# chriscoey/Hypatia.jl

Hardware: AMD Instinct MI355X
Metric: IPM iterations/sec (+ ms per KKT solve): dense n=5000, PosSemidefTri side 200 (Float64, QRCholDense + CombinedStepper) (higher is better)
Workload: dtype f64

## Files before the change

### hypatia.jl_amd/_lib.py

```python
import ctypes
import os

import numpy as np

HERE = os.path.dirname(os.path.abspath(__file__))
LIB_PATH = os.environ.get("HYP_LIB_PATH") or os.path.join(HERE, "libhypatia_hip.so")

c_int, c_dbl, c_vp = ctypes.c_int, ctypes.c_double, ctypes.c_void_p
P = ctypes.POINTER

_lib = None
_ctx = None


class HypatiaHipError(RuntimeError):
    pass


SIGNATURES = {
    "hyp_ctx_create": [c_int, P(c_vp)],
    "hyp_ctx_destroy": [c_vp],
    "hyp_ctx_synchronize": [c_vp],
    "hyp_device_count": [P(c_int)],
    "hyp_get_timers": [c_vp, c_vp],
# ... 58 lines not shown
    "hyp_sys_step_directions": [c_vp, c_vp, c_vp, c_dbl, c_dbl, c_int, c_dbl, c_dbl, c_vp, c_vp, P(c_int), P(c_int), P(c_int), P(c_int), c_vp],
    "hyp_sys_set_comm": [c_vp, c_vp, c_vp, c_vp, ctypes.c_long],
    "hyp_comm_unique_id": [c_vp],
    "hyp_comm_init_rank": [c_vp, c_int, c_int, c_vp, P(c_vp)],
    "hyp_comm_destroy": [c_vp],
    "hyp_comm_allreduce": [c_vp, c_vp, ctypes.c_long, c_int],
    "hyp_sys_set_comm_rccl": [c_vp, c_vp],
    "hyp_sys_comm_stats": [c_vp, c_vp],
    "hyp_qrcp_factor": [c_vp, c_int, c_int, c_vp, c_int, c_vp, P(c_vp)],
    "hyp_qrcp_get": [c_vp, c_vp, c_vp, c_vp, c_vp],
    "hyp_qrcp_apply_q": [c_vp, c_int, c_vp],
    "hyp_qrcp_destroy": [c_vp],
    "hyp_sys_set_kshard": [c_vp, c_int, c_int],
    "hyp_sys_set_direction_rows": [c_vp, c_int],
    "hyp_sys_last_update_lhs_seconds": [c_vp, P(c_dbl)],
    "hyp_sys_bench_gemv": [c_vp, c_int, c_vp],
    "hyp_sys_search_alpha": [c_vp, c_vp, c_vp, c_vp, c_vp, c_vp, c_int, c_int, c_vp, c_int, c_int, c_dbl, c_dbl, c_int, c_dbl, c_vp,
                             P(c_int), P(c_dbl), P(c_int), P(c_int), P(c_dbl)],
    "hyp_sys_search_screen_stats": [c_vp, P(c_int), c_vp, c_vp],
    "hyp_sys_search_alpha_resident": [c_vp, c_int, c_int, c_vp, c_int, c_int, c_dbl, c_dbl, c_int, c_dbl, c_vp,
                                      P(c_int), P(c_dbl), P(c_int), P(c_int), P(c_dbl)],
    "hyp_sys_check_cone_points": [c_vp, c_vp, c_dbl, c_dbl, c_int, c_dbl, P(c_int), P(c_dbl), P(c_int), P(c_dbl)],
    "hyp_sys_residual_products": [c_vp, c_vp, c_vp, c_vp, c_vp, c_vp, c_vp],
    "hyp_sys_residual_products2": [c_vp, c_vp, c_vp, c_vp, c_dbl, c_vp, c_vp, c_vp, c_vp],
    "hyp_sys_set_comm_layout": [c_vp, c_int, c_int],
    "hyp_sys_comm_hist": [c_vp, c_vp],
    "hyp_sys_comm_times": [c_vp, c_vp],
    "hyp_sys_allreduce_host": [c_vp, c_vp, c_int, c_int],
    "hyp_sys_load_model": [c_vp, c_vp, c_vp, c_vp, c_vp],
    "hyp_sys_update_lhs": [c_vp, P(c_int), P(c_int), P(c_int), c_vp],
    "hyp_sys_get_directions": [c_vp, c_vp, c_vp, c_dbl, c_dbl, c_int, c_dbl, c_dbl, P(c_dbl), P(c_int)],
    "hyp_sys_assemble_lhs": [c_vp, P(c_int)],
    "hyp_sys_factor_lhs": [c_vp, P(c_int), P(c_int)],
    "hyp_sys_lhs_export_dev": [c_vp, c_vp],
    "hyp_sys_lhs_import_dev": [c_vp, c_vp],
    "hyp_sys_set_lhs": [c_vp, c_vp],
    "hyp_sys_potrs": [c_vp, c_vp],
    "hyp_sys_block_hess_prod": [c_vp, c_vp, c_vp],
    "hyp_sys_mul_G": [c_vp, c_int, c_dbl, c_vp, c_dbl, c_vp],
    "hyp_sys_get_lhs": [c_vp, c_vp],
    "hyp_dense_gemm": [c_vp, c_int, c_int, c_int, c_int, c_int, c_dbl, c_vp, c_int, c_vp, c_int, c_dbl, c_vp, c_int],
    "hyp_dense_syrk": [c_vp, c_int, c_int, c_vp, c_int, c_vp, c_int],
    "hyp_dense_potrf": [c_vp, c_int, c_vp, c_int, P(c_int)],
    "hyp_dense_posdef_solve": [c_vp, c_int, c_vp, c_int, c_vp, c_int, c_int, P(c_int), P(c_int), P(c_int)],
    "hyp_dense_posv": [c_vp, c_int, c_vp, c_int, c_vp, P(c_int)],
    "hyp_dense_posv_multi": [c_vp, c_int, c_vp, c_int, c_vp, c_int, c_int, P(c_int)],
    "hyp_dense_sysv_rook": [c_vp, c_int, c_vp, c_int, c_vp, c_int, c_int, P(c_int), c_vp, c_vp, c_vp, c_vp],
    "hyp_dense_lstsq_normal": [c_vp, c_int, c_int, c_vp, c_int, c_vp, c_vp, P(c_dbl), P(c_int)],
    "hyp_dense_gemv": [c_vp, c_int, c_int, c_int, c_dbl, c_vp, c_int, c_vp, c_dbl, c_vp],
    "hyp_dense_gemv_both": [c_vp, c_int, c_int, c_int, c_vp, c_int, c_vp, c_dbl, c_vp, c_vp, c_dbl, c_vp, P(c_int)],
    "hyp_bench_syrk": [c_vp, c_int, c_int, c_int, P(c_dbl)],
    "hyp_bench_potrf": [c_vp, c_int, c_int, P(c_dbl)],
    "hyp_bench_trsv": [c_vp, c_int, c_int, P(c_dbl), P(c_dbl)],
}


def load_library():
    global _lib
    if _lib is not None:
        return _lib
    if not os.path.exists(LIB_PATH):
        raise HypatiaHipError("libhypatia_hip.so is missing at %s: run __graft_entry__.build() "
                              "(hipcc --offload-arch=gfx950); there is no CPU fallback" % LIB_PATH)
    lib = ctypes.CDLL(LIB_PATH)
    for name, argtypes in SIGNATURES.items():
        fn = getattr(lib, name)
        fn.argtypes = argtypes
        fn.restype = c_int
    lib.hyp_last_error.argtypes = [c_vp]
    lib.hyp_last_error.restype = ctypes.c_char_p
    if os.environ.get("HYP_PROFILE"):
        lib = _ProfiledLib(lib)
    _lib = lib
    return lib


class _ProfiledLib:

    def __init__(self, lib):
        import time
        self._lib = lib
        self.stats = {}
        self._time = time.perf_counter

    def __getattr__(self, name):
        fn = getattr(self._lib, name)
        if not name.startswith("hyp_") or name == "hyp_last_error":
            return fn
        stats, clock = self.stats, self._time

        def wrapped(*a):
            t0 = clock()
            r = fn(*a)
            st = stats.setdefault(name, [0, 0.0])
            st[0] += 1
            st[1] += clock() - t0
            return r
        wrapped.__name__ = name
        setattr(self, name, wrapped)
        return wrapped

    def report(self):
        rows = sorted(self.stats.items(), key=lambda kv: -kv[1][1])
        return "\n".join("%-36s calls %6d  total %9.3f ms  avg %8.1f us" % (k, v[0], v[1] * 1e3, v[1] / v[0] * 1e6) for k, v in rows)

    def reset(self):
# ... 52 lines not shown
```

### hypatia.jl_amd/csrc/capi.hip

```cpp
#include <unistd.h>
#include "../../include/hypatia_hip.h"
#include "syssolver.hpp"
#include <chrono>
#include <cstring>

using namespace hyp;

struct hyp_ctx { Ctx c; hyp_ctx(int d) : c(d) {} };
struct hyp_cone { hyp_ctx* ctx; Cone* cone; };
struct hyp_sys { hyp_ctx* ctx; SysSolver* s; };
struct hyp_symindef { hyp_ctx* ctx; SymIndefSys* s; };
struct hyp_comm { hyp_ctx* ctx; void* nccl; int nranks, rank; };
namespace hyp {
struct QrcpFact;
QrcpFact* qrcp_create(Ctx& c, int m, int n, const double* hA, int lda, const double* hb);
void qrcp_get(QrcpFact* f, int* jpvt, double* R, double* rdiag, double* qtb);
void qrcp_apply_q(QrcpFact* f, bool trans, double* hx);
void qrcp_destroy(QrcpFact* f);
}
struct hyp_qrcp { hyp_ctx* ctx; hyp::QrcpFact* f; };

namespace hyp {
void rccl_allreduce_inplace(void* comm, double* d_buf, long count, int op, hipStream_t st);
void rccl_unique_id(char* out128);
// ... 1096 lines not shown
      const double v = (double)(s >> 11) * (1.0 / 9007199254740992.0) - 0.5;
      h[j * n + i] = h[i * n + j] = (i == j) ? (double)n : v;
    }
  for (auto& v : hx) { s ^= s << 13; s ^= s >> 7; s ^= s << 17; v = (double)(s >> 11) * (1.0 / 9007199254740992.0) - 0.5; }
  c.h2d(dA.p, h.data(), h.size() * 8);
  c.h2d(dx0.p, hx.data(), hx.size() * 8);
  potrf_upper_batched(c, n, dA.d(), n, 0, 1, dinv.d(), dinfo.i());
  c.d2h(c.h_info, dinfo.p, sizeof(int));
  c.sync();
  HYP_REQUIRE(c.h_info[0] == 0, "bench_trsv: factorization failed");
  hipEvent_t e0, e1;
  HYP_CHECK(hipEventCreate(&e0)); HYP_CHECK(hipEventCreate(&e1));
  TriSolvePlan tri;
  float tb = 0, t1 = 0, t2 = 0, t3 = 0;
  for (int r = 0; r <= reps; ++r) {
    float ms = 0;
    tri.invalidate();
    HYP_CHECK(hipEventRecord(e0, c.stream));
    tri.build(c, n, dA.d(), n, dinv.d());
    HYP_CHECK(hipEventRecord(e1, c.stream));
    HYP_CHECK(hipEventSynchronize(e1));
    HYP_CHECK(hipEventElapsedTime(&ms, e0, e1));
    if (r > 0) tb += ms;
    c.d2d(dx.p, dx0.p, (size_t)3 * n * 8);
    HYP_CHECK(hipEventRecord(e0, c.stream));
    tri.solve_both(c, dA.d(), n, dx.d(), n, 1);
    HYP_CHECK(hipEventRecord(e1, c.stream));
    HYP_CHECK(hipEventSynchronize(e1));
    HYP_CHECK(hipEventElapsedTime(&ms, e0, e1));
    if (r > 0) t1 += ms;
    if (x_out && r == reps) c.d2h(x_out, dx.p, (size_t)n * 8);
    c.d2d(dx.p, dx0.p, (size_t)3 * n * 8);
    HYP_CHECK(hipEventRecord(e0, c.stream));
    tri.solve_both(c, dA.d(), n, dx.d(), n, 2);
    HYP_CHECK(hipEventRecord(e1, c.stream));
    HYP_CHECK(hipEventSynchronize(e1));
    HYP_CHECK(hipEventElapsedTime(&ms, e0, e1));
    if (r > 0) t2 += ms;
    if (x_out && r == reps) c.d2h(x_out + n, dx.p, (size_t)2 * n * 8);
    c.d2d(dx.p, dx0.p, (size_t)3 * n * 8);
    HYP_CHECK(hipEventRecord(e0, c.stream));
    tri.solve_both(c, dA.d(), n, dx.d(), n, 3);
    HYP_CHECK(hipEventRecord(e1, c.stream));
    HYP_CHECK(hipEventSynchronize(e1));
    HYP_CHECK(hipEventElapsedTime(&ms, e0, e1));
    if (r > 0) t3 += ms;
    if (x_out && r == reps) c.d2h(x_out + 3 * n, dx.p, (size_t)3 * n * 8);
  }
  c.sync();
  ms_out4[0] = tb / reps; ms_out4[1] = t1 / reps; ms_out4[2] = t2 / reps; ms_out4[3] = t3 / reps;
  (void)hipEventDestroy(e0); (void)hipEventDestroy(e1);
  API_END(ctx)
}
int hyp_bench_syrk(hyp_ctx* ctx, int N, int K, int reps, double* ms_out) {
  API_BEGIN
  Ctx& c = ctx->c;
  DBuf dA((size_t)K * N * 8), dC((size_t)N * N * 8);
  std::vector<double> h((size_t)K * N);
  uint64_t s = 88172645463325252ULL;
  for (auto& v : h) { s ^= s << 13; s ^= s >> 7; s ^= s << 17; v = (double)(s >> 11) * (1.0 / 9007199254740992.0) * 2.0 - 1.0; }
  c.h2d(dA.p, h.data(), h.size() * 8);
  c.sync();
  GemmArgs g{};
  g.M = N; g.N = N; g.K = K; g.A = dA.d(); g.lda = K; g.B = dA.d(); g.ldb = K; g.C = dC.d(); g.ldc = N;
  g.alpha = 1; g.beta = 0; g.tri = GEMM_UPPER; g.krange = KR_ALL; g.batch = 1; g.tag = 1;
  gemm(c, true, g);
  c.sync();
  hipEvent_t e0, e1;
  HYP_CHECK(hipEventCreate(&e0)); HYP_CHECK(hipEventCreate(&e1));
  float ms = 0;
  const char* gap = getenv("HYP_BENCH_SYRK_GAP_US");
  if (gap && atoi(gap) > 0) {
    for (int r = 0; r < reps; ++r) {
      c.sync();
      usleep(atoi(gap));
      HYP_CHECK(hipEventRecord(e0, c.stream));
      gemm(c, true, g);
      HYP_CHECK(hipEventRecord(e1, c.stream));
      const char* burst = getenv("HYP_BENCH_SYRK_BURST");
      const int nb = burst ? std::min(atoi(burst), 8) : 0;
      hipEvent_t eb[9];
      for (int b = 0; b < nb; ++b) {
        gemm(c, true, g);
        HYP_CHECK(hipEventCreate(&eb[b]));
        HYP_CHECK(hipEventRecord(eb[b], c.stream));
      }
      HYP_CHECK(hipEventSynchronize(nb ? eb[nb - 1] : e1));
      float t = 0;
      HYP_CHECK(hipEventElapsedTime(&t, e0, e1));
      ms += t;
      if (nb) {
        fprintf(stderr, "burst after %s us idle: %.3f", gap, t);
        for (int b = 0; b < nb; ++b) {
          float tb = 0;
          HYP_CHECK(hipEventElapsedTime(&tb, b ? eb[b - 1] : e1, eb[b]));
          fprintf(stderr, " %.3f", tb);
        }
        fprintf(stderr, " ms\n");
        for (int b = 0; b < nb; ++b) (void)hipEventDestroy(eb[b]);
      }
    }
  } else {
    HYP_CHECK(hipEventRecord(e0, c.stream));
    for (int r = 0; r < reps; ++r) gemm(c, true, g);
    HYP_CHECK(hipEventRecord(e1, c.stream));
    HYP_CHECK(hipEventSynchronize(e1));
// ... 9 lines not shown
```

### hypatia.jl_amd/csrc/dense.hip

```cpp
#include <malloc.h>
#include "tds_small.hpp"
#include "hyp_internal.hpp"

#include <fcntl.h>
#include <sys/file.h>
#include <sys/stat.h>
#include <unistd.h>

namespace hyp {

void gemm(Ctx& c, bool transa, GemmArgs a) { HYP_CHECK(gemm_f64_launch(c.stream, transa, a, &c.gemm_scratch)); }

void potrf_diag_launch(hipStream_t st, bool factor, bool invert, int batch, int nblocks, double* A, long lda, long strideA, int n, int k0,
                       double* dinv, long strideD, int* info, int own_cu_lds = 0);
int potrf_diag_own_cu_lds();
void potrf_panel_solve_launch(hipStream_t st, int batch, double* A, long lda, long strideA, int k0, int mcols);
void potrf_diag_mfma_launch(hipStream_t st, int batch, double* A, long lda, long strideA, int n, int k0, int* info, int own_cu_lds,
                            double* tinv = nullptr, long tinv_stride = 0, bool prev_update = false);
bool potrf_tinv_on();
bool potrf_diag_prev_ok();
int potrf_diag_mfma_own_cu_lds();
void potrf_panel_mfma_launch(hipStream_t st, int batch, double* A, long lda, long strideA, int k0, int mcols, int coff = 0,
                             const double* tinv = nullptr, long tinv_stride = 0);

// ... 792 lines not shown
      for (int g = 0; g < 4; ++g) {
        Rs[(rowA + 4 * g) * 16 + li] = rA[g];
        Rs[(rowB + 4 * g) * 16 + li] = rB[g];
      }
      __syncthreads();
      tdr_product<LOWER>(dop, nb, wv, Rs, xA, xB);
    }
    __syncthreads();
#pragma unroll
    for (int g = 0; g < 4; ++g) {
      Xs[(rowA + 4 * g) * 16 + li] = xA[g];
      Xs[(rowB + 4 * g) * 16 + li] = xB[g];
    }
    __syncthreads();
    for (int e = tid; e < NB * 16; e += 256) {
      const int k = e & (NB - 1), c = e >> 7;
      if (k < nb && c0 + c < nrhs) X[(long)(c0 + c) * ldx + k] = Xs[k * 16 + c];
    }
    __syncthreads();
  }
}

void trsm_upper_left_fwd_batched(Ctx& c, int n, int nrhs, const double* U, long ldu, long strideU, const double* dinv, long strideD,
                                 double* X, long ldx, long strideX, int batch) {
  if (n <= 0 || nrhs <= 0 || batch <= 0) return;
  const int nblk = (n + NB - 1) / NB;
  const int refine = std::max(1, trsm_refine_steps());
  for (int kb = 0; kb < nblk; ++kb) {
    const int k0 = kb * NB, nb = std::min(NB, n - k0), m = n - k0 - nb;
    hipLaunchKernelGGL(trsm_diag_refined_fwd_batched_kernel, dim3((nrhs + 16 * TDR_CH - 1) / (16 * TDR_CH), batch), dim3(256), 0, c.stream, U + (long)k0 * ldu + k0, ldu,
                       strideU, dinv + (long)kb * DINV_BLK, strideD, nb, X + k0, ldx, strideX, nrhs, refine);
    HYP_CHECK(hipGetLastError());
    if (m > 0) {
      GemmArgs u{};
      u.M = m; u.N = nrhs; u.K = nb; u.A = U + (long)(k0 + nb) * ldu + k0; u.lda = ldu; u.strideA = strideU;
      u.B = X + k0; u.ldb = ldx; u.strideB = strideX; u.C = X + k0 + nb; u.ldc = ldx; u.strideC = strideX;
      u.alpha = -1; u.beta = 1; u.batch = batch;
      gemm(c, true, u);
    }
  }
}

__global__ void place_dinv_kernel(const double* __restrict__ dinv, long strideD, double* __restrict__ Uinv, long ldi, long strideI,
                                  int n) {
  const int b = blockIdx.z;
  const int l = blockIdx.y;
  const int i = blockIdx.x * blockDim.x + threadIdx.x;
  if (i >= n || l >= n) return;
  double v = 0.0;
  if (i / NB == l / NB) v = dinv[(long)b * strideD + (long)(l / NB) * DINV_BLK + (long)(l % NB) * NB + (i % NB)];
  Uinv[(long)b * strideI + (long)l * ldi + i] = v;
}

void trtri_upper_batched(Ctx& c, int n, const double* U, long ldu, long strideU, const double* dinv, long strideD, double* Uinv,
                         long ldi, long strideI, int batch, DBuf* ws_override) {
  if (n <= 0 || batch <= 0) return;
  hipLaunchKernelGGL(place_dinv_kernel, dim3((n + 127) / 128, n, batch), dim3(128), 0, c.stream, dinv, strideD, Uinv, ldi, strideI, n);
  HYP_CHECK(hipGetLastError());
  const int nblk = (n + NB - 1) / NB;
  if (nblk == 1) return;
  DBuf& ws = ws_override ? *ws_override : c.work_tri;
  ws.ensure((size_t)batch * n * NB * sizeof(double));
  for (int jb = 1; jb < nblk; ++jb) {
    const int j0 = jb * NB, nb = std::min(NB, n - j0);
    GemmArgs t{};
    t.M = j0; t.N = nb; t.K = nb; t.A = U + (long)j0 * ldu; t.lda = ldu; t.strideA = strideU;
    t.B = dinv + (long)jb * DINV_BLK; t.ldb = NB; t.strideB = strideD;
    t.C = ws.d(); t.ldc = n; t.strideC = (long)n * NB; t.alpha = 1; t.beta = 0; t.krange = KR_LE_N; t.batch = batch;
    gemm(c, false, t);
    GemmArgs u{};
    u.M = j0; u.N = nb; u.K = j0; u.A = Uinv; u.lda = ldi; u.strideA = strideI;
    u.B = ws.d(); u.ldb = n; u.strideB = (long)n * NB;
    u.C = Uinv + (long)j0 * ldi; u.ldc = ldi; u.strideC = strideI; u.alpha = -1; u.beta = 0; u.krange = KR_GE_M; u.batch = batch;
    gemm(c, false, u);
  }
}

__global__ __launch_bounds__(256) void coldot_kernel(int m, int ncols, int mode, const double* __restrict__ M, long ld,
                                                     const double* __restrict__ v, const double* base, double alpha, double* out) {
  const int j = blockIdx.x * 4 + (threadIdx.x >> 6);
  if (j >= ncols) return;
  const int lane = threadIdx.x & 63;
  int i0 = 0, i1 = m;
  if (mode == 1) i1 = min(j + 1, m);
  else if (mode == 2) i0 = min(j, m);
  const double* a = M + (long)j * ld;
  double s0 = 0.0, s1 = 0.0, s2 = 0.0, s3 = 0.0;
  int i = i0 + lane;
  for (; i + 192 < i1; i += 256) {
    const double a0 = a[i], a1 = a[i + 64], a2 = a[i + 128], a3 = a[i + 192];
    s0 += a0 * v[i];
    s1 += a1 * v[i + 64];
    s2 += a2 * v[i + 128];
    s3 += a3 * v[i + 192];
  }
  for (; i < i1; i += 64) s0 += a[i] * v[i];
  double s = (s0 + s1) + (s2 + s3);
#pragma unroll
  for (int off = 32; off > 0; off >>= 1) s += __shfl_down(s, off);
  if (lane == 0) out[j] = (base ? base[j] : 0.0) + alpha * s;
}

__global__ __launch_bounds__(256) void coldot_batched_kernel(int m, int ncols, int mode, const double* __restrict__ M, long ld,
                                                             const double* __restrict__ v, const double* base, double alpha, double* out) {
  const int j = blockIdx.x * 4 + (threadIdx.x >> 6);
  if (j >= ncols) return;
  const int lane = threadIdx.x & 63;
  int i0 = 0, i1 = m;
// ... 62 lines not shown
    const double v1 = phase == 0 ? ((i & 1) ? -1.0 : 1.0) : t[n + r0 + i];
    s0 = fma(a, v0, s0);
    s1 = fma(a, v1, s1);
  }
#pragma unroll
  for (int off = 32; off > 0; off >>= 1) {
    s0 += __shfl_down(s0, off);
    s1 += __shfl_down(s1, off);
  }
  if (lane != 0) return;
  if (phase == 0) {
    t[J] = s0;
    t[n + J] = s1;
  } else {
    const double e0 = fabs(1.0 - s0), e1 = fabs(((j & 1) ? -1.0 : 1.0) - s1);
    double m = e0 > e1 ? e0 : e1;
    if (!(e0 == e0) || !(e1 == e1)) m = __longlong_as_double(0x7ff8000000000000LL);
    atomicMax(out, (unsigned long long)__double_as_longlong(m));
  }
}

void TriSolvePlan::measure_quality(Ctx& c, const double* U, long ldu) {
  probe_ws.ensure((size_t)(2 * n + 2) * sizeof(double));
  double* t = probe_ws.d();
  unsigned long long* out = reinterpret_cast<unsigned long long*>(t + 2 * n);
  c.zero(out, sizeof(unsigned long long));
  const dim3 grid((n + 3) / 4), blk(256);
  hipLaunchKernelGGL(plan_probe_kernel, grid, blk, 0, c.stream, 0, n, sb, Binv.d(), U, ldu, t, out);
  hipLaunchKernelGGL(plan_probe_kernel, grid, blk, 0, c.stream, 1, n, sb, Binv.d(), U, ldu, t, out);
  HYP_CHECK(hipGetLastError());
  c.d2h(c.h_pinned + 200, out, sizeof(double));
  c.sync();
  rho = c.h_pinned[200];
}

void TriSolvePlan::build(Ctx& c, int n_, const double* U, long ldu, const double* dinv) {
  n = 0;
  sb = c.trsv_plan_sb(n_);
  static const int refine_env = [] { const char* e = getenv("HYP_TRSV_REFINE"); return e ? atoi(e) : -1; }();
  refine_req = refine_env >= 0 ? refine_env : 2;
  refine = refine_req;
  rho = -1.0;
  if (sb <= 0 || n_ <= 0) return;
  const int nsb = (n_ + sb - 1) / sb;
  const size_t blk = (size_t)sb * sb;
  Binv.ensure(nsb * blk * sizeof(double));
  BinvT.ensure(nsb * blk * sizeof(double));
  UT.ensure((size_t)n_ * n_ * sizeof(double));
  work.ensure((size_t)2 * sb * sizeof(double));
  const int nfull = n_ / sb, last = n_ - nfull * sb;
  const long strideU = (long)sb * (ldu + 1), strideD = (long)(sb / NB) * DINV_BLK;
  const bool split = (nfull > 0 && last > 0);
  hipEvent_t e0 = c.aux_event(0), e1 = c.aux_event(1);
  if (split) {
    work2.ensure((size_t)last * NB * sizeof(double));
    HYP_CHECK(hipEventRecord(e0, c.stream));
    HYP_CHECK(hipStreamWaitEvent(c.stream2, e0, 0));
    {
      StreamSwap on_helper(c);
      dev_transpose(c, n_, n_, U, ldu, UT.d(), n_, 1, 0, 0);
      trtri_upper_batched(c, last, U + (long)nfull * strideU, ldu, 0, dinv + (long)nfull * strideD, 0, Binv.d() + nfull * blk, sb, 0, 1, &work2);
      dev_transpose(c, last, last, Binv.d() + nfull * blk, sb, BinvT.d() + nfull * blk, sb, 1, 0, 0);
      HYP_CHECK(hipEventRecord(e1, c.stream));
    }
  }
  if (nfull > 0) trtri_upper_batched(c, sb, U, ldu, strideU, dinv, strideD, Binv.d(), sb, (long)blk, nfull);
  if (!split && last > 0) {
    trtri_upper_batched(c, last, U + (long)nfull * strideU, ldu, 0, dinv + (long)nfull * strideD, 0, Binv.d() + nfull * blk, sb, 0, 1);
    dev_transpose(c, last, last, Binv.d() + nfull * blk, sb, BinvT.d() + nfull * blk, sb, 1, 0, 0);
  }
  if (nfull > 0) dev_transpose(c, sb, sb, Binv.d(), sb, BinvT.d(), sb, nfull, (long)blk, (long)blk);
  if (!split) dev_transpose(c, n_, n_, U, ldu, UT.d(), n_, 1, 0, 0);
  if (split) HYP_CHECK(hipStreamWaitEvent(c.stream, e1, 0));
  n = n_;
  static const int adapt_sel = [] { const char* e = getenv("HYP_TRSV_ADAPT"); return e ? atoi(e) : 3; }();
  const bool adapt = adapt_sel == 1 || (adapt_sel == 2 && owner_class == 0) || (adapt_sel == 3 && owner_class == 1);
  static const double adapt_tol = [] { const char* e = getenv("HYP_TRSV_ADAPT_TOL"); return e ? atof(e) : 1e-10; }();
  ++c.plan_builds;
  if (adapt && refine_req >= 2) {
    measure_quality(c, U, ldu);
    static const bool dbg = [] { const char* e = getenv("HYP_TRSV_ADAPT_DBG"); return e && e[0] == '1'; }();
    if (dbg) fprintf(stderr, "[solve plan] n = %d, super-blocks of %d: rho = %.3e\n", n, sb, rho);
    if (rho == rho && rho <= adapt_tol) { refine = 1; ++c.plan_builds_one_step; }
  }
  ol_prepare(c, ldu);
}

void TriSolvePlan::solve(Ctx& c, const double* U, long ldu, bool trans, double* x) {
  if (ol_usable(c, ldu, 1)) { ol_sweep(c, U, trans ? 0 : 1, x, 0, nullptr, 1); return; }
  const int nsb = (n + sb - 1) / sb;
  const size_t blk = (size_t)sb * sb;
  double* t = work.d();
  double* e = work.d() + sb;
  for (int s = 0; s < nsb; ++s) {
    const int b = trans ? s : nsb - 1 - s;
    const int r0 = b * sb, m = std::min(sb, n - r0);
    double* xb = x + r0;
    const double* Dm = trans ? U + (long)r0 * ldu + r0 : UT.d() + (long)r0 * n + r0;
    const long ldd = trans ? ldu : n;
    const double* Bm = (trans ? Binv.d() : BinvT.d()) + b * blk;
    const int mode = trans ? 1 : 2;
    if (refine == 0) {
      coldot(c, m, m, mode, Bm, sb, xb, nullptr, 1.0, t);
      HYP_CHECK(hipMemcpyAsync(xb, t, (size_t)m * sizeof(double), hipMemcpyDeviceToDevice, c.stream));
    } else {
      coldot(c, m, m, mode, Bm, sb, xb, nullptr, 1.0, t);
      for (int it = 0; it < refine; ++it) {
        coldot(c, m, m, mode, Dm, ldd, t, xb, -1.0, e);
        coldot(c, m, m, mode, Bm, sb, e, t, 1.0, it + 1 == refine ? xb : t);
      }
    }
    if (trans) {
      const int rest = n - (r0 + m);
      coldot(c, m, rest, 0, U + (long)(r0 + m) * ldu + r0, ldu, xb, x + r0 + m, -1.0, x + r0 + m);
    } else {
      coldot(c, m, r0, 0, UT.d() + r0, n, xb, x, -1.0, x);
    }
  }
  HYP_CHECK(hipGetLastError());
}

template <int NC>
__global__ __launch_bounds__(256) void coldotn_kernel(int m, int ncols, int mode, const double* __restrict__ M, long ld,
                                                      const double* __restrict__ v, long ldv, const double* base, long ldb, double alpha,
                                                      double* out, long ldo) {
  const int j = blockIdx.x * 4 + (threadIdx.x >> 6);
// ... 422 lines not shown
```

### hypatia.jl_amd/csrc/hyp_internal.hpp

```cpp
#pragma once
#include <hip/hip_runtime.h>
#include <stdint.h>
#include <string>
#include <vector>
#include <utility>
#include <stdexcept>
#include "gemm_f64.hpp"

namespace hyp {

struct HipError : std::runtime_error {
  int code;
  HipError(int c, const std::string& m) : std::runtime_error(m), code(c) {}
};

#define HYP_CHECK(expr)                                                                         \
  do {                                                                                          \
    hipError_t e_ = (expr);                                                                     \
    if (e_ != hipSuccess)                                                                       \
      throw hyp::HipError(-(int)e_ - 1000, std::string(#expr) + ": " + hipGetErrorString(e_) +  \
                                                " at " __FILE__ ":" + std::to_string(__LINE__)); \
  } while (0)

#define HYP_REQUIRE(cond, msg)                                                     \
// ... 117 lines not shown
  }
};

struct StreamSwap {
  Ctx& c;
  explicit StreamSwap(Ctx& ctx) : c(ctx) { std::swap(c.stream, c.stream2); std::swap(c.gemm_scratch, c.gemm_scratch2); std::swap(c.potrf_tinv, c.potrf_tinv2); }
  ~StreamSwap() { std::swap(c.stream, c.stream2); std::swap(c.gemm_scratch, c.gemm_scratch2); std::swap(c.potrf_tinv, c.potrf_tinv2); }
  StreamSwap(const StreamSwap&) = delete;
  StreamSwap& operator=(const StreamSwap&) = delete;
};

struct Ctx::Lane {
  hipStream_t s = nullptr;
  GemmScratch gs;
  DBuf tinv;
  hipEvent_t done = nullptr;
};

struct LaneSwitch {
  Ctx& c;
  int i;
  explicit LaneSwitch(Ctx& ctx, int lane) : c(ctx), i(lane) { flip(); }
  ~LaneSwitch() { flip(); }
  LaneSwitch(const LaneSwitch&) = delete;
  LaneSwitch& operator=(const LaneSwitch&) = delete;
 private:
  void flip() {
    if (i == 1) { std::swap(c.stream, c.stream2); std::swap(c.gemm_scratch, c.gemm_scratch2); std::swap(c.potrf_tinv, c.potrf_tinv2); }
    else if (i >= 2) { Ctx::Lane& L = c.lane(i); std::swap(c.stream, L.s); std::swap(c.gemm_scratch, L.gs); std::swap(c.potrf_tinv, L.tinv); }
  }
};
void fork_lanes(Ctx& c, int nlanes);
void join_lanes(Ctx& c, int nlanes);


void potrf_upper_batched(Ctx& c, int n, double* A, long lda, long strideA, int batch, double* dinv, int* d_info, int kb_stop = -1);
bool potrf_split_ok(int n, int n1);
void schur_split_begin(Ctx& c, int n, int K, const double* A, long lda, double* C, double* F, int n1, int* d_info, hipStream_t lane,
                       hipEvent_t left_ready, hipEvent_t left_done);
void schur_split_finish(Ctx& c, int n, const double* C, double* F, int n1, double* dinv, int* d_info, hipEvent_t left_done);
void potrf_invert_diag_blocks(Ctx& c, int n, double* A , long lda, long strideA, int batch, double* dinv,
                              long strideD = 0 );
constexpr long DINV_BLK = 2L * NB * NB;
inline size_t dinv_elems(int n) { return (size_t)((n + NB - 1) / NB) * DINV_BLK; }

void trsv_upper(Ctx& c, int n, const double* U, long ldu, const double* dinv, bool trans, double* x);
int trsm_refine_steps();
void trsm_upper_left(Ctx& c, int n, int nrhs, const double* U, long ldu, const double* dinv, bool trans, double* X,
                     long ldx, double* work );
void trsm_upper_left_fwd_batched(Ctx& c, int n, int nrhs, const double* U, long ldu, long strideU, const double* dinv, long strideD,
                                 double* X, long ldx, long strideX, int batch);
struct TriSolvePlan {
  int n = 0, sb = 0, refine = 2;
  DBuf Binv, BinvT, UT, work, work2, work_n;
  bool ready(int n_) const { return n == n_ && n_ > 0; }
  void invalidate() { n = 0; }
  void build(Ctx& c, int n_, const double* U, long ldu, const double* dinv);
  DBuf ol_rounds[4], ol_arena;
  bool ol_ok = false;
  bool ol_have[4] = {false, false, false, false};
  int ol_n = 0, ol_sb = 0, ol_set = 0;
  long ol_ldu = 0, ol_asz = 0;
  int ol_first[4][3] = {}, ol_n0[4][3] = {}, ol_n1[4][3] = {};
  void ol_prepare(Ctx& c, long ldu);
  int refine_req = 2;
  int owner_class = 0;
  double rho = -1.0;
  DBuf probe_ws;
  void measure_quality(Ctx& c, const double* U, long ldu);
  bool ol_fit[4] = {false, false, false, false};
  static bool ol_fits(Ctx& c, int nr);
  bool ol_usable(const Ctx& c, long ldu, int nr) const { return ol_ok && nr >= 1 && nr <= 3 && ol_fit[nr] && c.persistent_ok && refine >= 0 && refine <= 3 && ol_have[refine] && ldu == ol_ldu && c.stream == c.stream_primary; }
  void ol_sweep(Ctx& c, const double* U, int which, double* x, long ldx, double* x3, int nr);
  void solve_both(Ctx& c, const double* U, long ldu, double* x, long ldx, int nr, double* x3 = nullptr);
  void solve(Ctx& c, const double* U, long ldu, bool trans, double* x);
  void solve_multi(Ctx& c, const double* U, long ldu, bool trans, double* x, long ldx, int nr);
  void solve_multi3(Ctx& c, const double* U, long ldu, bool trans, double* x, long ldx, double* x3);
  void solve_n(Ctx& c, const double* U, long ldu, bool trans, double* x, long ldx, int nc);
};
struct BKFact {
  int n = 0;
  int n_2x2 = 0;
  DBuf dd, de, blk, perm;
  DBuf state, wl, tmp, tr;
  DBuf guard;
  int k0_used = 0;
  int guard_trimmed = 0;
  int factor(Ctx& c, int n_, double* A, long lda, double* dinv);
  int factor_from(Ctx& c, int n_, double* A, long lda, double* dinv, int k0);
  double* gather(Ctx& c, const double* x, long ldx, int nr);
  void dsolve(Ctx& c, double* y, long ldy, int nr);
  void scatter(Ctx& c, const double* y, double* x, long ldx, int nr);
  void solve(Ctx& c, const double* U, long ldu, const double* dinv, double* x, long ldx, int nr, DBuf& trsm_work);
};
int bk_after_failed_cholesky(Ctx& c, BKFact& bk, int n, double* A, long lda, double* dinv, int* d_info_scratch, int chol_info,
                             const double* A_src, long ld_src);
void gemv_multi(Ctx& c, bool trans, int m, int n, int nr, double alpha, const double* A, long lda, const double* X, long ldx, double beta,
                double* Y, long ldy);
bool gemv_both_ok(int m, int n, const double* A, long lda);
void gemv_both(Ctx& c, int m, int n, int nr, const double* A, long lda, const double* Xn, long ldxn, double beta_n, double* Yn, long ldyn,
               const double* Xt, long ldxt, double beta_t, double* Yt, long ldyt);
void trtri_upper_batched(Ctx& c, int n, const double* U, long ldu, long strideU, const double* dinv, long strideD,
                         double* Uinv, long ldi, long strideI, int batch, DBuf* ws_override = nullptr);

void gemv(Ctx& c, bool trans, int m, int n, double alpha, const double* A, long lda, const double* x, double beta,
          double* y);

void dev_dot(Ctx& c, int n, const double* x, const double* y, double* d_out);
struct DotSpecs {
  int count = 0;
  int n[8];
  const double* x[8];
  const double* y[8];
  double* out[8];
  void add(int n_, const double* x_, const double* y_, double* out_) { n[count] = n_; x[count] = x_; y[count] = y_; out[count] = out_; ++count; }
};
void dev_dots(Ctx& c, const DotSpecs& sp);
struct ZeroSlots {
  int count = 0;
  double* p[16];
  void add(double* q) { p[count++] = q; }
};
void dev_zero_slots(Ctx& c, const ZeroSlots& z);
void dev_axpby(Ctx& c, int n, double a, const double* x, double b, double* y);
void dev_scale_copy(Ctx& c, int n, double a, const double* x, double* y);
void dev_transpose(Ctx& c, int m, int n, const double* A, long lda, double* B, long ldb, int batch, long strideA,
                   long strideB);
void dev_fill_identity(Ctx& c, int n, double* A, long lda);
void dev_symmetrize_from_upper(Ctx& c, int n, double* A, long lda, int batch, long stride);
void dev_zero_strict_lower(Ctx& c, int n, double* A, long lda, int batch, long stride);

void svec_unpack(Ctx& c, int side, int ncols, const double* arr, long ldarr, double* mats);
void svec_unpack_grouped(Ctx& c, int side, int ngroups, int group, const double* arr, long ldg, long ldarr, double* mats);
void svec_pack(Ctx& c, int side, int ncols, const double* mats, double* arr, long ldarr, double scale);

void gemm(Ctx& c, bool transa, GemmArgs a);

}
```

### include/hypatia_hip.h

```cpp
#ifndef HYPATIA_HIP_H
#define HYPATIA_HIP_H
#ifdef __cplusplus
extern "C" {
#endif

typedef struct hyp_ctx hyp_ctx;
typedef struct hyp_cone hyp_cone;
typedef struct hyp_sys hyp_sys;

int hyp_ctx_create(int device, hyp_ctx** out);
int hyp_ctx_destroy(hyp_ctx* ctx);
int hyp_ctx_synchronize(hyp_ctx* ctx);
const char* hyp_last_error(hyp_ctx* ctx);
int hyp_device_count(int* out);
int hyp_get_timers(hyp_ctx* ctx, double* out10);
int hyp_reset_timers(hyp_ctx* ctx);
int hyp_get_kernel_stats(hyp_ctx* ctx, double* out8);
int hyp_ctx_bk_stats(hyp_ctx* ctx, long long* out3);
int hyp_ctx_plan_stats(hyp_ctx* ctx, long long* out2);

int hyp_cone_create_nonnegative(hyp_ctx* ctx, int dim, hyp_cone** out);
int hyp_cone_create_possemideftri(hyp_ctx* ctx, int dim, hyp_cone** out);
int hyp_cone_create_possemideftri_complex(hyp_ctx* ctx, int dim, hyp_cone** out);
int hyp_cone_create_epinormspectral(hyp_ctx* ctx, int d1, int d2, int use_dual, hyp_cone** out);
// ... 72 lines not shown
int hyp_sys_get_directions2(hyp_sys* sys, double* dir_vecs, const double* rhs_vecs, double mu, double tau, int max_ref_steps,
                            double res_norm_cutoff, double min_impr_tol, double* res_norms, int* n_solves);
int hyp_sys_check_cone_points(hyp_sys* sys, const double* cand_ztsk, double min_prox, double prox_bound, int use_max_prox, double nup1,
                              int* accept, double* prox, int* n_loaded, double* irtmu);
int hyp_sys_step_directions(hyp_sys* sys, const double* point_vec, const double* residuals, double tau_residual, double mu, int max_ref_steps,
                            double res_norm_cutoff, double min_impr_tol, double* dir_vecs4, double* res_norms4, int* n_solves,
                            int* use_sqrt_hess_cones_out, int* info, int* used_fallback, double* sol_const_out );
int hyp_sys_set_comm(hyp_sys* sys, int (*allreduce)(void* user, long count, int op), void* user, void* device_staging, long capacity_doubles);
typedef struct hyp_comm hyp_comm;
int hyp_comm_unique_id(char* out128);
int hyp_comm_init_rank(hyp_ctx* ctx, int nranks, int rank, const char* id128, hyp_comm** out);
int hyp_comm_destroy(hyp_comm* comm);
int hyp_comm_allreduce(hyp_comm* comm, void* device_buf, long count, int op);
int hyp_sys_set_comm_rccl(hyp_sys* sys, hyp_comm* comm);
int hyp_sys_set_comm_layout(hyp_sys* sys, int rank, int world);
int hyp_sys_comm_hist(hyp_sys* sys, long long* out16);
int hyp_sys_comm_times(hyp_sys* sys, double* out16);
int hyp_sys_set_kshard(hyp_sys* sys, int rank, int world);
int hyp_sys_comm_stats(hyp_sys* sys, double* out2);
int hyp_sys_set_direction_rows(hyp_sys* sys, int x_rows_only);
int hyp_sys_last_update_lhs_seconds(hyp_sys* sys, double* out);
int hyp_sys_bench_gemv(hyp_sys* sys, int reps, double* ms_out4);
int hyp_sys_search_alpha(hyp_sys* sys, const double* point_ztsk, const double* dir_cent, const double* dir_pred, const double* dir_centadj,
                         const double* dir_predadj, int unadj_only, int cent_only, const double* alpha_sched, int nsched, int start,
                         double min_prox, double prox_bound, int use_max_prox, double nup1, double* cand_ztsk, int* accepted_index,
                         double* prox, int* n_trials, int* n_loaded, double* irtmu);
int hyp_sys_search_alpha_resident(hyp_sys* sys, int unadj_only, int cent_only, const double* alpha_sched, int nsched, int start, double min_prox,
                                  double prox_bound, int use_max_prox, double nup1, double* cand_ztsk, int* accepted_index, double* prox,
                                  int* n_trials, int* n_loaded, double* irtmu);
int hyp_sys_search_screen_stats(hyp_sys* sys, int* usable, long long* screens, long long* rejected);
int hyp_sys_get_lhs(hyp_sys* sys, double* out_nmpxnmp);

int hyp_dense_gemm(hyp_ctx* ctx, int transa, int upper, int M, int N, int K, double alpha, const double* A, int lda,
                   const double* B, int ldb, double beta, double* C, int ldc);
int hyp_dense_syrk(hyp_ctx* ctx, int N, int K, const double* A, int lda, double* C, int ldc);
int hyp_dense_potrf(hyp_ctx* ctx, int n, double* A, int lda, int* info);
int hyp_dense_posv(hyp_ctx* ctx, int n, double* A, int lda, double* x, int* info);
int hyp_dense_posv_multi(hyp_ctx* ctx, int n, double* A, int lda, double* X, int nrhs, int ldx, int* info);
int hyp_dense_sysv_rook(hyp_ctx* ctx, int n, double* A, int lda, double* x, int nrhs, int ldx, int* info, int* perm, int* blk,
                        double* d, double* e);
int hyp_dense_posdef_solve(hyp_ctx* ctx, int n, double* A, int lda, double* x, int nrhs, int ldx, int* info, int* used_fallback, int* bk_start);
typedef struct hyp_qrcp hyp_qrcp;
int hyp_qrcp_factor(hyp_ctx* ctx, int m, int n, const double* A, int lda, const double* rhs, hyp_qrcp** out);
int hyp_qrcp_get(hyp_qrcp* q, int* jpvt, double* R, double* rdiag, double* qtb);
int hyp_qrcp_apply_q(hyp_qrcp* q, int trans, double* vec);
int hyp_qrcp_destroy(hyp_qrcp* q);
int hyp_dense_lstsq_normal(hyp_ctx* ctx, int m, int n, const double* A, int lda, const double* b, double* x, double* rcond_est, int* info);
int hyp_dense_gemv(hyp_ctx* ctx, int trans, int m, int n, double alpha, const double* A, int lda, const double* x, double beta,
                   double* y);
int hyp_dense_gemv_both(hyp_ctx* ctx, int m, int n, int nr, const double* A, int lda, const double* Xn, double beta_n, double* Yn,
                        const double* Xt, double beta_t, double* Yt, int* used_fused);
int hyp_bench_potrf(hyp_ctx* ctx, int n, int reps, double* ms_out);
int hyp_bench_trsv(hyp_ctx* ctx, int n, int reps, double* ms_out4, double* x_out);
int hyp_bench_syrk(hyp_ctx* ctx, int N, int K, int reps, double* ms_out);

#ifdef __cplusplus
}
#endif
#endif
```

Baseline: 57.71.

## Replace chained block trtri with three-kernel strip inversion in solve-plan build

Adds a new triangular-inverse path that builds the blocked upper-triangular inverse with three launches: one placing the diagonal-block inverses, one MFMA kernel filling a workspace of off-diagonal products, and one strip kernel that chains the block-row recurrence in LDS. It replaces the per-block chain of GEMM launches used when building the triangular-solve plan. Both the full-size and remainder blocks go into a single grouped launch, and the transpose overlaps on the helper stream. The path is on by default (env HYP_TRTRI_ONE_LAUNCH). It adds workspace memory and LDS use, and falls back to the old chain when there are more than 10 or fewer than 3 blocks.

```diff
diff --git a/hypatia.jl_amd/_lib.py b/hypatia.jl_amd/_lib.py
--- a/hypatia.jl_amd/_lib.py
+++ b/hypatia.jl_amd/_lib.py
@@ -134,6 +134,8 @@
     "hyp_bench_syrk": [c_vp, c_int, c_int, c_int, P(c_dbl)],
     "hyp_bench_potrf": [c_vp, c_int, c_int, P(c_dbl)],
     "hyp_bench_trsv": [c_vp, c_int, c_int, P(c_dbl), P(c_dbl)],
+    "hyp_dense_trtri_upper": [c_vp, c_int, c_vp, c_int, c_vp, c_int, c_int, ctypes.c_long, ctypes.c_long, c_int],
+    "hyp_bench_plan_build": [c_vp, c_int, c_int, P(c_dbl)],
 }
 
 
diff --git a/hypatia.jl_amd/csrc/capi.hip b/hypatia.jl_amd/csrc/capi.hip
--- a/hypatia.jl_amd/csrc/capi.hip
+++ b/hypatia.jl_amd/csrc/capi.hip
@@ -1172,6 +1172,64 @@
   (void)hipEventDestroy(e0); (void)hipEventDestroy(e1);
   API_END(ctx)
 }
+int hyp_dense_trtri_upper(hyp_ctx* ctx, int n, const double* U, int ldu, double* Uinv, int ldi, int batch, long strideU, long strideI,
+                          int form) {
+  API_BEGIN
+  Ctx& c = ctx->c;
+  HYP_REQUIRE(n >= 1 && batch >= 1 && ldu >= n && ldi >= n && (form == 0 || form == 1), "trtri_upper: sizes");
+  HYP_REQUIRE(batch == 1 || (strideU >= (long)ldu * n && strideI >= (long)ldi * n), "trtri_upper: strides smaller than a matrix");
+  const size_t nU = (size_t)(batch - 1) * strideU + (size_t)ldu * n, nI = (size_t)(batch - 1) * strideI + (size_t)ldi * n;
+  const long strideD = (long)dinv_elems(n);
+  DBuf dU(nU * 8), dI(nI * 8), dinv((size_t)batch * strideD * 8);
+  c.h2d(dU.p, U, nU * 8);
+  c.h2d(dI.p, Uinv, nI * 8);
+  potrf_invert_diag_blocks(c, n, dU.d(), ldu, strideU, batch, dinv.d(), strideD);
+  trtri_upper_batched(c, n, dU.d(), ldu, strideU, dinv.d(), strideD, dI.d(), ldi, strideI, batch, nullptr, form);
+  c.d2h(Uinv, dI.p, nI * 8);
+  c.sync();
+  API_END(ctx)
+}
+int hyp_bench_plan_build(hyp_ctx* ctx, int n, int reps, double* ms_out) {
+  API_BEGIN
+  Ctx& c = ctx->c;
+  HYP_REQUIRE(n >= 1 && reps >= 1, "bench_plan_build: sizes");
+  HYP_REQUIRE(c.trsv_plan_sb(n) > 0, "bench_plan_build: a factor of this size has no solve plan");
+  DBuf dA((size_t)n * n * 8), dinv(dinv_elems(n) * 8), dinfo(64);
+  std::vector<double> h((size_t)n * n);
+  uint64_t s = 88172645463325252ULL;
+  for (long j = 0; j < n; ++j)
+    for (long i = 0; i <= j; ++i) {
+      s ^= s << 13; s ^= s >> 7; s ^= s << 17;
+      const double v = (double)(s >> 11) * (1.0 / 9007199254740992.0) - 0.5;
+      h[j * n + i] = h[i * n + j] = (i == j) ? (double)n : v;
+    }
+  c.h2d(dA.p, h.data(), h.size() * 8);
+  potrf_upper_batched(c, n, dA.d(), n, 0, 1, dinv.d(), dinfo.i());
+  c.d2h(c.h_info, dinfo.p, sizeof(int));
+  c.sync();
+  HYP_REQUIRE(c.h_info[0] == 0, "bench_plan_build: factorization failed");
+  hipEvent_t e0, e1;
+  HYP_CHECK(hipEventCreate(&e0)); HYP_CHECK(hipEventCreate(&e1));
+  for (int form = 0; form < 2; ++form) {
+    TriSolvePlan tri;
+    tri.trtri_form = form;
+    float total = 0;
+    for (int r = 0; r <= reps; ++r) {
+      float ms = 0;
+      tri.invalidate();
+      HYP_CHECK(hipEventRecord(e0, c.stream));
+      tri.build(c, n, dA.d(), n, dinv.d());
+      HYP_CHECK(hipEventRecord(e1, c.stream));
+      HYP_CHECK(hipEventSynchronize(e1));
+      HYP_CHECK(hipEventElapsedTime(&ms, e0, e1));
+      if (r > 0) total += ms;
+    }
+    c.sync();
+    ms_out[form] = total / reps;
+  }
+  (void)hipEventDestroy(e0); (void)hipEventDestroy(e1);
+  API_END(ctx)
+}
 int hyp_bench_syrk(hyp_ctx* ctx, int N, int K, int reps, double* ms_out) {
   API_BEGIN
   Ctx& c = ctx->c;
diff --git a/hypatia.jl_amd/csrc/dense.hip b/hypatia.jl_amd/csrc/dense.hip
--- a/hypatia.jl_amd/csrc/dense.hip
+++ b/hypatia.jl_amd/csrc/dense.hip
@@ -868,8 +868,8 @@
   Uinv[(long)b * strideI + (long)l * ldi + i] = v;
 }
 
-void trtri_upper_batched(Ctx& c, int n, const double* U, long ldu, long strideU, const double* dinv, long strideD, double* Uinv,
-                         long ldi, long strideI, int batch, DBuf* ws_override) {
+void trtri_upper_chain(Ctx& c, int n, const double* U, long ldu, long strideU, const double* dinv, long strideD, double* Uinv,
+                       long ldi, long strideI, int batch, DBuf* ws_override) {
   if (n <= 0 || batch <= 0) return;
   hipLaunchKernelGGL(place_dinv_kernel, dim3((n + 127) / 128, n, batch), dim3(128), 0, c.stream, dinv, strideD, Uinv, ldi, strideI, n);
   HYP_CHECK(hipGetLastError());
@@ -1038,6 +1038,28 @@
   const long strideU = (long)sb * (ldu + 1), strideD = (long)(sb / NB) * DINV_BLK;
   const bool split = (nfull > 0 && last > 0);
   hipEvent_t e0 = c.aux_event(0), e1 = c.aux_event(1);
+  const bool one_launch = trtri_form < 0 ? trtri_one_launch_on() : trtri_form == 1;
+  if (one_launch) {
+    if (split) {
+      HYP_CHECK(hipEventRecord(e0, c.stream));
+      HYP_CHECK(hipStreamWaitEvent(c.stream2, e0, 0));
+      StreamSwap on_helper(c);
+      dev_transpose(c, n_, n_, U, ldu, UT.d(), n_, 1, 0, 0);
+    }
+    TrtriProb pr[2];
+    int np = 0;
+    if (nfull > 0) pr[np++] = TrtriProb{sb, nfull, U, ldu, strideU, dinv, strideD, Binv.d(), sb, (long)blk, BinvT.d(), sb, (long)blk};
+    if (last > 0)
+      pr[np++] = TrtriProb{last, 1, U + (long)nfull * strideU, ldu, 0, dinv + (long)nfull * strideD, 0, Binv.d() + nfull * blk, sb, 0,
+                           BinvT.d() + nfull * blk, sb, 0};
+    trtri_upper_multi(c, pr, np, 1, split);
+    if (split) {
+      HYP_CHECK(hipEventRecord(e1, c.stream2));
+      HYP_CHECK(hipStreamWaitEvent(c.stream, e1, 0));
+    } else {
+      dev_transpose(c, n_, n_, U, ldu, UT.d(), n_, 1, 0, 0);
+    }
+  } else {
   if (split) {
     work2.ensure((size_t)last * NB * sizeof(double));
     HYP_CHECK(hipEventRecord(e0, c.stream));
@@ -1045,19 +1067,20 @@
     {
       StreamSwap on_helper(c);
       dev_transpose(c, n_, n_, U, ldu, UT.d(), n_, 1, 0, 0);
-      trtri_upper_batched(c, last, U + (long)nfull * strideU, ldu, 0, dinv + (long)nfull * strideD, 0, Binv.d() + nfull * blk, sb, 0, 1, &work2);
+      trtri_upper_chain(c, last, U + (long)nfull * strideU, ldu, 0, dinv + (long)nfull * strideD, 0, Binv.d() + nfull * blk, sb, 0, 1, &work2);
       dev_transpose(c, last, last, Binv.d() + nfull * blk, sb, BinvT.d() + nfull * blk, sb, 1, 0, 0);
       HYP_CHECK(hipEventRecord(e1, c.stream));
     }
   }
-  if (nfull > 0) trtri_upper_batched(c, sb, U, ldu, strideU, dinv, strideD, Binv.d(), sb, (long)blk, nfull);
+  if (nfull > 0) trtri_upper_chain(c, sb, U, ldu, strideU, dinv, strideD, Binv.d(), sb, (long)blk, nfull, nullptr);
   if (!split && last > 0) {
-    trtri_upper_batched(c, last, U + (long)nfull * strideU, ldu, 0, dinv + (long)nfull * strideD, 0, Binv.d() + nfull * blk, sb, 0, 1);
+    trtri_upper_chain(c, last, U + (long)nfull * strideU, ldu, 0, dinv + (long)nfull * strideD, 0, Binv.d() + nfull * blk, sb, 0, 1, nullptr);
     dev_transpose(c, last, last, Binv.d() + nfull * blk, sb, BinvT.d() + nfull * blk, sb, 1, 0, 0);
   }
   if (nfull > 0) dev_transpose(c, sb, sb, Binv.d(), sb, BinvT.d(), sb, nfull, (long)blk, (long)blk);
   if (!split) dev_transpose(c, n_, n_, U, ldu, UT.d(), n_, 1, 0, 0);
   if (split) HYP_CHECK(hipStreamWaitEvent(c.stream, e1, 0));
+  }
   n = n_;
   static const int adapt_sel = [] { const char* e = getenv("HYP_TRSV_ADAPT"); return e ? atoi(e) : 3; }();
   const bool adapt = adapt_sel == 1 || (adapt_sel == 2 && owner_class == 0) || (adapt_sel == 3 && owner_class == 1);
diff --git a/hypatia.jl_amd/csrc/hyp_internal.hpp b/hypatia.jl_amd/csrc/hyp_internal.hpp
--- a/hypatia.jl_amd/csrc/hyp_internal.hpp
+++ b/hypatia.jl_amd/csrc/hyp_internal.hpp
@@ -193,6 +193,7 @@
                                  double* X, long ldx, long strideX, int batch);
 struct TriSolvePlan {
   int n = 0, sb = 0, refine = 2;
+  int trtri_form = -1;
   DBuf Binv, BinvT, UT, work, work2, work_n;
   bool ready(int n_) const { return n == n_ && n_ > 0; }
   void invalidate() { n = 0; }
@@ -242,7 +243,18 @@
 void gemv_both(Ctx& c, int m, int n, int nr, const double* A, long lda, const double* Xn, long ldxn, double beta_n, double* Yn, long ldyn,
                const double* Xt, long ldxt, double beta_t, double* Yt, long ldyt);
 void trtri_upper_batched(Ctx& c, int n, const double* U, long ldu, long strideU, const double* dinv, long strideD,
-                         double* Uinv, long ldi, long strideI, int batch, DBuf* ws_override = nullptr);
+                         double* Uinv, long ldi, long strideI, int batch, DBuf* ws_override = nullptr, int form = -1);
+void trtri_upper_chain(Ctx& c, int n, const double* U, long ldu, long strideU, const double* dinv, long strideD,
+                       double* Uinv, long ldi, long strideI, int batch, DBuf* ws_override);
+struct TrtriProb {
+  int n, batch;
+  const double* U; long ldu, strideU;
+  const double* dinv; long strideD;
+  double* Uinv; long ldi, strideI;
+  double* UinvT; long ldt, strideT;
+};
+void trtri_upper_multi(Ctx& c, const TrtriProb* probs, int nprobs, int form = -1, bool place_on_helper = false);
+bool trtri_one_launch_on();
 
 void gemv(Ctx& c, bool trans, int m, int n, double alpha, const double* A, long lda, const double* x, double beta,
           double* y);
diff --git a/hypatia.jl_amd/csrc/trtri_strips.hip b/hypatia.jl_amd/csrc/trtri_strips.hip
--- /dev/null
+++ b/hypatia.jl_amd/csrc/trtri_strips.hip
@@ -0,0 +1,244 @@
+#include "hyp_internal.hpp"
+
+#include <algorithm>
+#include <cstdlib>
+
+namespace hyp {
+
+namespace {
+
+constexpr int TT_MAXG = 2;
+constexpr int TT_STRIP = 16;
+constexpr int TT_THREADS = 512;
+constexpr int TT_MAX_NBLK = 10;
+constexpr long TT_WS_BLK = (long)NB * NB;
+
+struct TrtriGroup {
+  int n, nblk, batch, first;
+  const double* U; long ldu, strideU;
+  const double* dinv; long strideD;
+  double* Uinv; long ldi, strideI;
+  double* UinvT; long ldt, strideT;
+  double* ws; long strideW;
+};
+struct TrtriLaunch {
+  int ngroups, members;
+  TrtriGroup g[TT_MAXG];
+};
+
+__device__ __forceinline__ int chain_tile(int J, int batch) { return ((long)J * batch < 192) ? 64 : 128; }
+
+__global__ void trtri_place_kernel(TrtriLaunch L) {
+  const int mem = blockIdx.z;
+  const TrtriGroup& g = L.g[(L.ngroups > 1 && mem >= L.g[1].first) ? 1 : 0];
+  const int b = mem - g.first;
+  const int l = blockIdx.y;
+  const int i = blockIdx.x * blockDim.x + threadIdx.x;
+  if (i >= g.n || l >= g.n) return;
+  const int bi = i / NB, bl = l / NB;
+  const double* __restrict__ dinv = g.dinv + (long)b * g.strideD + (long)bl * DINV_BLK;
+  if (bi >= bl) g.Uinv[(long)b * g.strideI + (long)l * g.ldi + i] = (bi == bl) ? dinv[(long)(l % NB) * NB + (i % NB)] : 0.0;
+  if (g.UinvT && bi <= bl) g.UinvT[(long)b * g.strideT + (long)l * g.ldt + i] = (bi == bl) ? dinv[(long)(i % NB) * NB + (l % NB)] : 0.0;
+}
+
+__global__ __launch_bounds__(256) void trtri_ws_kernel(TrtriLaunch L) {
+  const int mem = blockIdx.y;
+  const TrtriGroup& g = L.g[(L.ngroups > 1 && mem >= L.g[1].first) ? 1 : 0];
+  const int b = mem - g.first;
+  int J = 1;
+  while ((J + 1) * J <= (int)blockIdx.x) ++J;
+  if (J >= g.nblk) return;
+  const int m0 = 64 * ((int)blockIdx.x - J * (J - 1));
+  const int j0 = J * NB, nb = min(NB, g.n - j0);
+  const int lane = threadIdx.x & 63, w = threadIdx.x >> 6, fr = lane & 15, fk = lane >> 4;
+  if (32 * w >= nb) return;
+  const int bt = chain_tile(J, g.batch);
+  const int kend = min(nb, bt == 64 ? (w >= 2 ? 128 : 64) : 128);
+  const int nch = ((kend + 15) / 16) * 4;
+  const double* __restrict__ A = g.U + (long)b * g.strideU + (long)j0 * g.ldu + m0 + fr;
+  const double* __restrict__ D = g.dinv + (long)b * g.strideD + (long)J * DINV_BLK;
+  const double* Dn[2];
+  double nmask[2];
+#pragma unroll
+  for (int t = 0; t < 2; ++t) {
+    const int nl = 32 * w + 16 * t + fr;
+    Dn[t] = D + (long)min(nl, nb - 1) * NB;
+    nmask[t] = nl < nb ? 1.0 : 0.0;
+  }
+  d4_t acc[2][4];
+#pragma unroll
+  for (int t = 0; t < 2; ++t)
+#pragma unroll
+    for (int i = 0; i < 4; ++i) acc[t][i] = (d4_t){0.0, 0.0, 0.0, 0.0};
+#pragma unroll 8
+  for (int c = 0; c < nch; ++c) {
+    const int k = 4 * c + fk, kc = min(k, kend - 1);
+    const double kmask = k < kend ? 1.0 : 0.0;
+    double af[4], bf[2];
+#pragma unroll
+    for (int i = 0; i < 4; ++i) af[i] = A[(long)kc * g.ldu + 16 * i] * kmask;
+#pragma unroll
+    for (int t = 0; t < 2; ++t) bf[t] = Dn[t][kc] * (nmask[t] * kmask);
+#pragma unroll
+    for (int t = 0; t < 2; ++t)
+#pragma unroll
+      for (int i = 0; i < 4; ++i) acc[t][i] = __builtin_amdgcn_mfma_f64_16x16x4f64(bf[t], af[i], acc[t][i], 0, 0, 0);
+  }
+  double* __restrict__ W = g.ws + (long)b * g.strideW + (long)(J * (J - 1) / 2) * TT_WS_BLK;
+  const double alpha = 1.0;
+#pragma unroll
+  for (int t = 0; t < 2; ++t)
+#pragma unroll
+    for (int r = 0; r < 4; ++r) {
+      const int nl = 32 * w + 16 * t + fk + 4 * r;
+      if (nl >= nb) continue;
+#pragma unroll
+      for (int i = 0; i < 4; ++i) W[(long)(m0 + 16 * i + fr) * NB + nl] = alpha * acc[t][i][r];
+    }
+}
+
+__device__ __forceinline__ void strip_load16(double (&buf)[32], int half, const double* __restrict__ Wcol, int k0, int fk, int klast) {
+#pragma unroll
+  for (int c = 0; c < 16; ++c) buf[16 * half + c] = Wcol[(long)min(k0 + 64 * half + 4 * c + fk, klast) * NB];
+}
+
+__global__ __launch_bounds__(TT_THREADS) void trtri_strip_kernel(TrtriLaunch L, double alpha) {
+  extern __shared__ __attribute__((aligned(16))) double Ls[];
+  const int mem = blockIdx.x % L.members, s = blockIdx.x / L.members;
+  const TrtriGroup& g = L.g[(L.ngroups > 1 && mem >= L.g[1].first) ? 1 : 0];
+  const int nblk = g.nblk;
+  if (s >= (nblk - 1) * (NB / TT_STRIP)) return;
+  const int b = mem - g.first;
+  const int i0 = s * TT_STRIP, ib = i0 / NB, kbase = ib * NB;
+  const int tid = threadIdx.x, lane = tid & 63, w = tid >> 6, fr = lane & 15, fk = lane >> 4;
+  {
+    const double* __restrict__ D = g.dinv + (long)b * g.strideD + (long)ib * DINV_BLK + (i0 - kbase);
+    for (int e = tid; e < NB * TT_STRIP; e += TT_THREADS) Ls[e] = D[(long)(e >> 4) * NB + (e & 15)];
+  }
+  __syncthreads();
+  const double* __restrict__ Wm = g.ws + (long)b * g.strideW + 16 * w + fr;
+  double* __restrict__ Um = g.Uinv + (long)b * g.strideI + i0 + fr;
+  double* __restrict__ Tm = g.UinvT ? g.UinvT + (long)b * g.strideT + (long)(i0 + fr) * g.ldt : nullptr;
+  const double* lsr = Ls + fk * TT_STRIP + fr;
+
+  int J = ib + 1;
+  int k = i0 & ~(chain_tile(J, g.batch) - 1);
+  double cur[32], nxt[32];
+  {
+    const double* Wc = Wm + (long)(J * (J - 1) / 2) * TT_WS_BLK;
+    strip_load16(nxt, 0, Wc, k, fk, J * NB - 1);
+    if ((k & 127) == 0) strip_load16(nxt, 1, Wc, k, fk, J * NB - 1);
+  }
+  d4_t acc = (d4_t){0.0, 0.0, 0.0, 0.0};
+  while (true) {
+#pragma unroll
+    for (int c = 0; c < 32; ++c) cur[c] = nxt[c];
+    const int kend = (k | 127) + 1;
+    const bool full = (kend - k) == 128;
+    const bool endJ = kend == J * NB;
+    int Jn = J, kn = kend;
+    if (endJ) { Jn = J + 1; kn = i0 & ~(chain_tile(Jn, g.batch) - 1); }
+    const bool more = Jn < nblk;
+    if (more) {
+      const double* Wc = Wm + (long)(Jn * (Jn - 1) / 2) * TT_WS_BLK;
+      strip_load16(nxt, 0, Wc, kn, fk, Jn * NB - 1);
+      if ((kn & 127) == 0) strip_load16(nxt, 1, Wc, kn, fk, Jn * NB - 1);
+    }
+    const double* la = lsr + (long)(k - kbase) * TT_STRIP;
+#pragma unroll
+    for (int c = 0; c < 16; ++c) acc = __builtin_amdgcn_mfma_f64_16x16x4f64(cur[c], la[4 * c * TT_STRIP], acc, 0, 0, 0);
+    if (full) {
+#pragma unroll
+      for (int c = 16; c < 32; ++c) acc = __builtin_amdgcn_mfma_f64_16x16x4f64(cur[c], la[4 * c * TT_STRIP], acc, 0, 0, 0);
+    }
+    if (endJ) {
+      const int j0 = J * NB, nb = min(NB, g.n - j0);
+#pragma unroll
+      for (int r = 0; r < 4; ++r) {
+        const int nl = 16 * w + fk + 4 * r;
+        if (nl >= nb) continue;
+        const double v = alpha * acc[r];
+        Um[(long)(j0 + nl) * g.ldi] = v;
+        if (Tm) Tm[j0 + nl] = v;
+        if (J + 1 < nblk) Ls[(long)(j0 - kbase + nl) * TT_STRIP + fr] = v;
+      }
+      acc = (d4_t){0.0, 0.0, 0.0, 0.0};
+      __syncthreads();
+    }
+    if (!more) break;
+    J = Jn; k = kn;
+  }
+}
+
+bool trtri_one_launch_env() {
+  static const bool on = [] { const char* e = getenv("HYP_TRTRI_ONE_LAUNCH"); return !(e && atoi(e) == 0); }();
+  return on;
+}
+
+size_t strip_lds_bytes(int nblk) { return (size_t)(nblk - 1) * NB * TT_STRIP * sizeof(double); }
+
+}
+
+void trtri_upper_multi(Ctx& c, const TrtriProb* probs, int nprobs, int form, bool place_on_helper) {
+  const bool one = form < 0 ? trtri_one_launch_env() : form == 1;
+  TrtriLaunch L{};
+  size_t ws_doubles = 0;
+  int max_n = 0, max_nblk = 0;
+  const TrtriProb* chain[8];
+  int nchain = 0;
+  HYP_REQUIRE(nprobs >= 0 && nprobs <= 8, "trtri_upper_multi: at most 8 problems");
+  for (int p = 0; p < nprobs; ++p) {
+    const TrtriProb& q = probs[p];
+    if (q.n <= 0 || q.batch <= 0) continue;
+    const int nblk = (q.n + NB - 1) / NB;
+    if (!one || nblk < 3 || nblk > TT_MAX_NBLK || L.ngroups == TT_MAXG) { chain[nchain++] = &q; continue; }
+    TrtriGroup& g = L.g[L.ngroups++];
+    g.n = q.n; g.nblk = nblk; g.batch = q.batch; g.first = L.members;
+    g.U = q.U; g.ldu = q.ldu; g.strideU = q.strideU; g.dinv = q.dinv; g.strideD = q.strideD;
+    g.Uinv = q.Uinv; g.ldi = q.ldi; g.strideI = q.strideI; g.UinvT = q.UinvT; g.ldt = q.ldt; g.strideT = q.strideT;
+    g.strideW = (long)(nblk * (nblk - 1) / 2) * TT_WS_BLK;
+    L.members += q.batch;
+    ws_doubles += (size_t)q.batch * g.strideW;
+    max_n = std::max(max_n, q.n);
+    max_nblk = std::max(max_nblk, nblk);
+  }
+  size_t chain_doubles = 0;
+  for (int p = 0; p < nchain; ++p) chain_doubles = std::max(chain_doubles, (size_t)chain[p]->batch * chain[p]->n * NB);
+  c.work_tri.ensure((ws_doubles + chain_doubles) * sizeof(double));
+  if (L.ngroups > 0) {
+    double* ws = c.work_tri.d() + chain_doubles;
+    for (int gi = 0; gi < L.ngroups; ++gi) { L.g[gi].ws = ws; ws += (size_t)L.g[gi].batch * L.g[gi].strideW; }
+    static const bool attr_ok = [] {
+      return hipFuncSetAttribute((const void*)trtri_strip_kernel, hipFuncAttributeMaxDynamicSharedMemorySize, (int)strip_lds_bytes(TT_MAX_NBLK)) == hipSuccess;
+    }();
+    HYP_REQUIRE(attr_ok, "trtri_strip_kernel: the device refused the strip kernel's LDS");
+    hipLaunchKernelGGL(trtri_place_kernel, dim3((max_n + 127) / 128, max_n, L.members), dim3(128), 0, place_on_helper ? c.stream2 : c.stream, L);
+    hipLaunchKernelGGL(trtri_ws_kernel, dim3(max_nblk * (max_nblk - 1), L.members), dim3(256), 0, c.stream, L);
+    hipLaunchKernelGGL(trtri_strip_kernel, dim3((max_nblk - 1) * (NB / TT_STRIP) * L.members), dim3(TT_THREADS), strip_lds_bytes(max_nblk), c.stream, L, -1.0);
+    HYP_CHECK(hipGetLastError());
+  }
+  for (int p = 0; p < nchain; ++p) {
+    const TrtriProb& q = *chain[p];
+    trtri_upper_chain(c, q.n, q.U, q.ldu, q.strideU, q.dinv, q.strideD, q.Uinv, q.ldi, q.strideI, q.batch, nullptr);
+    if (q.UinvT) dev_transpose(c, q.n, q.n, q.Uinv, q.ldi, q.UinvT, q.ldt, q.batch, q.strideI, q.strideT);
+  }
+}
+
+void trtri_upper_batched(Ctx& c, int n, const double* U, long ldu, long strideU, const double* dinv, long strideD, double* Uinv,
+                         long ldi, long strideI, int batch, DBuf* ws_override, int form) {
+  if (n <= 0 || batch <= 0) return;
+  const int nblk = (n + NB - 1) / NB;
+  const bool one = form < 0 ? trtri_one_launch_env() : form == 1;
+  if (!one || nblk < 3 || nblk > TT_MAX_NBLK) {
+    trtri_upper_chain(c, n, U, ldu, strideU, dinv, strideD, Uinv, ldi, strideI, batch, ws_override);
+    return;
+  }
+  TrtriProb q{};
+  q.n = n; q.batch = batch; q.U = U; q.ldu = ldu; q.strideU = strideU; q.dinv = dinv; q.strideD = strideD;
+  q.Uinv = Uinv; q.ldi = ldi; q.strideI = strideI;
+  trtri_upper_multi(c, &q, 1, 1);
+}
+
+bool trtri_one_launch_on() { return trtri_one_launch_env(); }
+
+}
diff --git a/include/hypatia_hip.h b/include/hypatia_hip.h
--- a/include/hypatia_hip.h
+++ b/include/hypatia_hip.h
@@ -148,6 +148,9 @@
                         const double* Xt, double beta_t, double* Yt, int* used_fused);
 int hyp_bench_potrf(hyp_ctx* ctx, int n, int reps, double* ms_out);
 int hyp_bench_trsv(hyp_ctx* ctx, int n, int reps, double* ms_out4, double* x_out);
+int hyp_dense_trtri_upper(hyp_ctx* ctx, int n, const double* U, int ldu, double* Uinv, int ldi, int batch, long strideU, long strideI,
+                          int form);
+int hyp_bench_plan_build(hyp_ctx* ctx, int n, int reps, double* ms_out);
 int hyp_bench_syrk(hyp_ctx* ctx, int N, int K, int reps, double* ms_out);
 
 #ifdef __cplusplus
```

New measurement: 59.56, median of 4. +3.2%, better.
